# andabi/parallel-wavenet-vocoder

Hardware: AMD Instinct MI355X
Metric: audio samples/sec, 4-flow IAF generation (higher is better)
Workload: dtype f32 via 3-term split-fp16 MFMA (fp32 accumulate, fp32 storage)

## Files before the change

### parallel-wavenet-vocoder_amd/csrc/pwv_f16x3.h

```cpp
#pragma once

#include "pwv_layer_common.h"

namespace pwv {

typedef float f32x2 __attribute__((ext_vector_type(2)));

template <int OFF, int N>
__device__ __forceinline__ void split8(const float (&x)[N], f16x8& hi, f16x8& lo) {
#pragma unroll
    for (int q = 0; q < 8; q += 2) {
        const f32x2 v = {x[OFF + q], x[OFF + q + 1]};
        const f16x2 h = __builtin_convertvector(v, f16x2);
        f32x2 r;
        asm("v_fma_mix_f32 %0, %1, -1.0, %2 op_sel:[0,0,0] op_sel_hi:[1,0,0]" : "=v"(r[0]) : "v"(h), "v"(v[0]));
        asm("v_fma_mix_f32 %0, %1, -1.0, %2 op_sel:[1,0,0] op_sel_hi:[1,0,0]" : "=v"(r[1]) : "v"(h), "v"(v[1]));
        const f16x2 l = __builtin_convertvector(r, f16x2);
        hi[q] = h[0];
        hi[q + 1] = h[1];
        lo[q] = l[0];
        lo[q + 1] = l[1];
    }
}

// ... 48 lines not shown
        f16x8 nh[4] = {ah[0], ah[1], ah[2], ah[3]};
        f16x8 nl[4] = {al[0], al[1], al[2], al[3]};
        if (s + 1 < S1) {
#pragma unroll
            for (int i = 0; i < NIT; ++i) {
                nh[i] = frag16<NS, NITTOT>(A, 0, IT0 + i * ITSTEP, s + 1, lane);
                nl[i] = frag16<NS, NITTOT>(A, 1, IT0 + i * ITSTEP, s + 1, lane);
            }
        } else {
            tail(nh, nl);
        }
        __builtin_amdgcn_sched_barrier(0);
        const f16x8 b_h = bh(s);
        const f16x8 b_l = bl(s);
#pragma unroll
        for (int i = 0; i < NIT; ++i)
            acc[IT0 + i * ITSTEP] = __builtin_amdgcn_mfma_f32_32x32x16_f16(ah[i], b_h, acc[IT0 + i * ITSTEP], 0, 0, 0);
#pragma unroll
        for (int i = 0; i < NIT; ++i)
            acc[IT0 + i * ITSTEP] = __builtin_amdgcn_mfma_f32_32x32x16_f16(ah[i], b_l, acc[IT0 + i * ITSTEP], 0, 0, 0);
#pragma unroll
        for (int i = 0; i < NIT; ++i)
            acc[IT0 + i * ITSTEP] = __builtin_amdgcn_mfma_f32_32x32x16_f16(al[i], b_h, acc[IT0 + i * ITSTEP], 0, 0, 0);
        extra(s);
        __builtin_amdgcn_sched_barrier(0);
#pragma unroll
        for (int i = 0; i < 4; ++i) {
            ah[i] = nh[i];
            al[i] = nl[i];
        }
    }
}

template <int NS, int S, int NIT, int IT0, int ITSTEP, int NITTOT>
__device__ __forceinline__ void frags_at(const f16x8* A, int lane, f16x8 (&h)[4], f16x8 (&l)[4]) {
#pragma unroll
    for (int i = 0; i < NIT; ++i) {
        h[i] = frag16<NS, NITTOT>(A, 0, IT0 + i * ITSTEP, S, lane);
        l[i] = frag16<NS, NITTOT>(A, 1, IT0 + i * ITSTEP, S, lane);
    }
}

template <int NS, int NIT, int IT0, int ITSTEP, int NITTOT>
__device__ __forceinline__ void first_frags(const f16x8* A, int lane, f16x8 (&h)[4], f16x8 (&l)[4]) {
#pragma unroll
    for (int i = 0; i < NIT; ++i) {
        h[i] = frag16<NS, NITTOT>(A, 0, IT0 + i * ITSTEP, 0, lane);
        l[i] = frag16<NS, NITTOT>(A, 1, IT0 + i * ITSTEP, 0, lane);
    }
}

}
```

### parallel-wavenet-vocoder_amd/csrc/pwv_head_f16x3.inc

```
            f32x16 accs[4];
#pragma unroll
            for (int it = 0; it < 4; ++it)
#pragma unroll
                for (int q = 0; q < 4; ++q) {
                    const f32x4 v = *reinterpret_cast<const f32x4*>(hb + kHBS + h * 64 + it * 16 + q * 4);
#pragma unroll
                    for (int e = 0; e < 4; ++e) accs[it][q * 4 + e] = v[e];
                }
#pragma unroll
            for (int r = 0; r < 16; ++r) o[16 + r] = gate_act(acc[1][r], acc[3][r]);
            split8<16>(o, oh[2], ol[2]);
            split8<24>(o, oh[3], ol[3]);
            first_frags<4, 4, 0, 1, 4>(HS, lane, ah, al);
            gemm16<4, 4, 0, 1, 4>(HS, lane, accs, ah, al, [&](int s) -> f16x8 { return oh[s]; },
                                  [&](int s) -> f16x8 { return ol[s]; }, no_extra,
                                  [&](f16x8(&nh)[4], f16x8(&nl)[4]) { first_frags<8, 4, 0, 1, 4>(H1, lane, nh, nl); });
#pragma unroll
            for (int it = 0; it < 4; ++it)
#pragma unroll
                for (int q = 0; q < 4; ++q) {
                    const f32x4 v = *reinterpret_cast<const f32x4*>(hb + kHB1 + h * 64 + it * 16 + q * 4);
#pragma unroll
                    for (int e = 0; e < 4; ++e) acc1[it][q * 4 + e] = v[e];
                }
            f16x8 sh[8], sl[8];
            {
                float r[64];
#pragma unroll
                for (int i = 0; i < 64; ++i) r[i] = fmaxf(accs[i >> 4][i & 15], 0.f);
                split8<0>(r, sh[0], sl[0]);
                split8<8>(r, sh[1], sl[1]);
                split8<16>(r, sh[2], sl[2]);
                split8<24>(r, sh[3], sl[3]);
                split8<32>(r, sh[4], sl[4]);
                split8<40>(r, sh[5], sl[5]);
                split8<48>(r, sh[6], sl[6]);
                split8<56>(r, sh[7], sl[7]);
            }
            gemm16<8, 4, 0, 1, 4>(H1, lane, acc1, ah, al, [&](int s) -> f16x8 { return sh[s]; },
                                  [&](int s) -> f16x8 { return sl[s]; }, no_extra, [](f16x8(&)[4], f16x8(&)[4]) {});
```

### parallel-wavenet-vocoder_amd/csrc/pwv_head_pp2.inc

```
                    for (int q = 0; q < Q; ++q) {
                        float part = 0.f;
                        const float* w2 = hb + kHW2 + (hq + q) * 64;
#pragma unroll
                        for (int i4 = 0; i4 < 16; ++i4) {
                            const f32x4 wv = *reinterpret_cast<const f32x4*>(w2 + 4 * i4);
#pragma unroll
                            for (int e = 0; e < 4; ++e) {
                                const int i = 4 * i4 + e;
                                part = fmaf(fmaxf(acc1[i >> 4][i & 15], 0.f), wv[e], part);
                            }
                        }
                        part += __shfl_xor(part, 32);
                        part += hb[kHW2 + 2 * Q * 64 + q];
                        PWV_HEAD_STORE(q, part);
                    }
```

### parallel-wavenet-vocoder_amd/csrc/pwv_layer_f16x3_body.inc

```
    static_assert(!HEAD || (GATED && !SKIP && !COND && !FIRST), "HEAD: plain last layer only");
    static_assert(!FOLD || FIRST, "FOLD: layer 0 of a scalar-input net only");
    static_assert(!STREAM || (SKIP ? !COND && !FIRST && !HEAD : FOLD == FIRST && (COND ? !HEAD && !(FIRST && GATED) : GATED == HEAD)),
                  "STREAM: folded layer 0, plain residual layer, last layer + head; COND: the last layer gated, its head a launch of its own; "
                  "SKIP: a residual or gated layer on row histories (layer 0 behind a streaming front), the head a launch of its own");
    constexpr int WAVES = 8;
    constexpr int kLds = HEAD ? kA1Size + kASSize + kHA1Size : layer_floats(SKIP, COND);
    constexpr int kCF = kLds + 4;
    constexpr int kHS = kA1Size;
    constexpr int kH1 = kA1Size + kASSize;
    __shared__ __attribute__((aligned(16))) float lds[kLds + (HEAD ? 0 : 4) + (FIRST ? 128 : 0)];

    const int tid = threadIdx.x;
    const int lane = tid & 63;
    const int wave = __builtin_amdgcn_readfirstlane(tid >> 6);
    const int h = lane >> 5;
    const int net = blockIdx.x % p.G;
    const int wg = blockIdx.x / p.G;
    const int nwg = gridDim.x / p.G;
    int* unit_counter = reinterpret_cast<int*>(&lds[HEAD ? 0 : kLds]);
#ifdef PWV_TRACE
    if (p.trace && tid == 0) {
        p.trace[4096 + blockIdx.x * 4 + 0] = __builtin_amdgcn_s_memtime();
        p.trace[4096 + 1024 + blockIdx.x * 2 + 0] = __builtin_amdgcn_s_memrealtime();
    }
// ... 170 lines not shown
                    *reinterpret_cast<f32x4*>(hw + g * 256) = v;
                }
            }
        }
        auto split_xc = [&](int s) {
            if (s == 0) { split8<0>(xc, bh[4], bl[4]); asm volatile("" : "+v"(bh[4]), "+v"(bl[4])); }
            if (s == 1) { split8<8>(xc, bh[5], bl[5]); asm volatile("" : "+v"(bh[5]), "+v"(bl[5])); }
            if (s == 2) { split8<16>(xc, bh[6], bl[6]); asm volatile("" : "+v"(bh[6]), "+v"(bl[6])); }
            if (s == 3) { split8<24>(xc, bh[7], bl[7]); asm volatile("" : "+v"(bh[7]), "+v"(bl[7])); }
        };
        auto split_xb = [&](int s) {
            if (s == 0) { split8<0>(rxb, bh[0], bl[0]); asm volatile("" : "+v"(bh[0]), "+v"(bl[0])); }
            if (s == 1) { split8<8>(rxb, bh[1], bl[1]); asm volatile("" : "+v"(bh[1]), "+v"(bl[1])); }
            if (s == 2) { split8<16>(rxb, bh[2], bl[2]); asm volatile("" : "+v"(bh[2]), "+v"(bl[2])); }
            if (s == 3) { split8<24>(rxb, bh[3], bl[3]); asm volatile("" : "+v"(bh[3]), "+v"(bl[3])); }
        };
        if constexpr (!FOLD) {
#pragma unroll
            for (int s = 0; s < 4; ++s) {
                if constexpr (COND) split_xb(s);
                else split_xc(s);
            }
        }

        auto bxh = [&](int s) -> f16x8 { return bh[s ^ 4]; };
        auto bxl = [&](int s) -> f16x8 { return bl[s ^ 4]; };
        auto bch = [&](int s) -> f16x8 { return ch[COND ? s : 0]; };
        auto bcl = [&](int s) -> f16x8 { return cl[COND ? s : 0]; };

        PWV_STAMP(3);
        float o[32];
        f16x8 oh[4], ol[4];
        f16x8 ah[4], al[4];

        if constexpr (FOLD) {
            if constexpr (COND) {
                first_frags<5, 2, 0, 2, 4>(AC, lane, ah, al);
                gemm16<5, 2, 0, 2, 4>(AC, lane, acc, ah, al, bch, bcl, no_extra,
                                      [&](f16x8(&nh)[4], f16x8(&nl)[4]) { first_frags<5, 2, 1, 2, 4>(AC, lane, nh, nl); });
                gemm16<5, 2, 1, 2, 4>(AC, lane, acc, ah, al, bch, bcl, no_extra, [](f16x8(&)[4], f16x8(&)[4]) {});
            }
            const f16x8* F0 = reinterpret_cast<const f16x8*>(p.fold0[net]);
            f16x8 fh[4], fl[4];
#pragma unroll
            for (int it = 0; it < 4; ++it) {
                fh[it] = F0[it * 64 + lane];
                fl[it] = F0[(4 + it) * 64 + lane];
            }
#pragma unroll
            for (int it = 0; it < 4; ++it) acc[it] = __builtin_amdgcn_mfma_f32_32x32x16_f16(fh[it], fb_h, acc[it], 0, 0, 0);
#pragma unroll
            for (int it = 0; it < 4; ++it) acc[it] = __builtin_amdgcn_mfma_f32_32x32x16_f16(fh[it], fb_l, acc[it], 0, 0, 0);
#pragma unroll
            for (int it = 0; it < 4; ++it) acc[it] = __builtin_amdgcn_mfma_f32_32x32x16_f16(fl[it], fb_h, acc[it], 0, 0, 0);
            if constexpr (!GATED) first_frags<4, 2, 0, 1, 2>(A2, lane, ah, al);
#pragma unroll
            for (int r = 0; r < 16; ++r) o[r] = gate_act(acc[0][r], acc[2][r]);
            split8<0>(o, oh[0], ol[0]);
            split8<8>(o, oh[1], ol[1]);
        } else {
        if constexpr (COND) {
            first_frags<5, 2, 0, 2, 4>(AC, lane, ah, al);
            gemm16<5, 2, 0, 2, 4>(AC, lane, acc, ah, al, bch, bcl, split_xc,
                                  [&](f16x8(&nh)[4], f16x8(&nl)[4]) { first_frags<8, 2, 0, 2, 4>(A1, lane, nh, nl); });
        } else {
            first_frags<8, 2, 0, 2, 4>(A1, lane, ah, al);
        }
        gemm16<8, 2, 0, 2, 4>(
            A1, lane, acc, ah, al, bxh, bxl,
            [&](int s) {
                if constexpr (!COND) split_xb(s);
            },
            [&](f16x8(&nh)[4], f16x8(&nl)[4]) {
                if constexpr (COND) first_frags<5, 2, 1, 2, 4>(AC, lane, nh, nl);
                else first_frags<8, 2, 1, 2, 4>(A1, lane, nh, nl);
            });
        PWV_STAMP(4);
        if constexpr (COND) {
            gemm16<5, 2, 1, 2, 4>(AC, lane, acc, ah, al, bch, bcl, no_extra,
                                  [&](f16x8(&nh)[4], f16x8(&nl)[4]) { first_frags<8, 2, 1, 2, 4>(A1, lane, nh, nl); });
        }
        gemm16<8, 2, 1, 2, 4>(
            A1, lane, acc, ah, al, bxh, bxl,
            [&](int s) {
                o[2 * s] = gate_act(acc[0][2 * s], acc[2][2 * s]);
                o[2 * s + 1] = gate_act(acc[0][2 * s + 1], acc[2][2 * s + 1]);
                asm volatile("" : "+v"(o[2 * s]), "+v"(o[2 * s + 1]));
                if (s == 3) {
                    split8<0>(o, oh[0], ol[0]);
                    asm volatile("" : "+v"(oh[0]), "+v"(ol[0]));
                }
                if (s == 7) {
                    split8<8>(o, oh[1], ol[1]);
                    asm volatile("" : "+v"(oh[1]), "+v"(ol[1]));
                }
            },
            [&](f16x8(&nh)[4], f16x8(&nl)[4]) {
                if constexpr (!GATED) first_frags<4, 2, 0, 1, 2>(A2, lane, nh, nl);
                else if constexpr (SKIP) first_frags<4, 2, 0, 1, 4>(AS, lane, nh, nl);
            });
        }

        PWV_STAMP(5);
        const int ooff = units_off(row, h, 64, u_begin);
        if constexpr (GATED && HEAD) {
            const float* hb = p.packed_head[net];
            const f16x8* HS = reinterpret_cast<const f16x8*>(&lds[kHS]);
            const f16x8* H1 = reinterpret_cast<const f16x8*>(&lds[kH1]);
            f32x16 acc1[4];
#include "pwv_head_f16x3.inc"
            load_x(next, rxb, rxc);
            const int Q = p.head_q;
            const int hq = h * Q;
#define PWV_HEAD_STORE(q, part) if (valid && h == 0) p.head_out[net][(size_t)row * Q + (q)] = (part)
#include "pwv_head_pp2.inc"
#undef PWV_HEAD_STORE
        } else if constexpr (GATED) {
            if constexpr (!SKIP) load_x(next, rxb, rxc);
            __builtin_amdgcn_sched_barrier(0);
#pragma unroll
            for (int r = 0; r < 16; ++r) o[16 + r] = gate_act(acc[1][r], acc[3][r]);
            if constexpr (SKIP) {
                split8<16>(o, oh[2], ol[2]);
                split8<24>(o, oh[3], ol[3]);
            }
            if (valid) {
#pragma unroll
                for (int g = 0; g < 8; ++g) {
                    f32x4 v = {o[4 * g], o[4 * g + 1], o[4 * g + 2], o[4 * g + 3]};
                    store_wt(out_rs, ooff + g * 1024, v);
                }
            }
        } else {
            f32x16 acc2[2];
#pragma unroll
            for (int it = 0; it < 2; ++it)
#pragma unroll
                for (int q = 0; q < 4; ++q) {
                    const f32x4 bd = *reinterpret_cast<const f32x4*>(&lds[kBD + h * 32 + it * 16 + q * 4]);
#pragma unroll
                    for (int e = 0; e < 4; ++e) acc2[it][q * 4 + e] = xc[it * 16 + q * 4 + e] + bd[e];
                }
            asm volatile("" : "+v"(acc2[0]), "+v"(acc2[1]));
            if constexpr (!SKIP) load_x(next, rxb, rxc);
            __builtin_amdgcn_sched_barrier(0);
// ... 81 lines not shown
```

### parallel-wavenet-vocoder_amd/csrc/pwv_layer_f32_body.inc

```
    static_assert(!FOLD || FIRST, "FOLD: layer 0 of a scalar-input net only");
    static_assert(!STREAM || (SKIP ? !COND && !FIRST && !HEAD : FOLD == FIRST && (COND ? !HEAD && !(FIRST && GATED) : GATED == HEAD)),
                  "STREAM: folded layer 0, plain residual layer, last layer + head; COND: the last layer gated, its head a launch of its own; "
                  "SKIP: a residual or gated layer on row histories (layer 0 behind a streaming front), the head a launch of its own");
    static_assert(!HEAD || (GATED && !SKIP && !COND && !FIRST), "HEAD: plain last layer only");
    static_assert(!FIRST || !SKIP, "FIRST: no skip accumulation");
    constexpr int WAVES = 8;
    constexpr int kLds = HEAD ? kA1Size + kASSize + kHA1Size : layer_floats(SKIP, COND);
    constexpr int kCF = kLds + 4;
    constexpr int kHS = kA1Size;
    constexpr int kH1 = kA1Size + kASSize;
    __shared__ __attribute__((aligned(16))) float lds[kLds + (HEAD ? 0 : 4) + (FIRST ? 128 : 0)];

    const int tid = threadIdx.x;
    const int lane = tid & 63;
    const int wave = __builtin_amdgcn_readfirstlane(tid >> 6);
    const int h = lane >> 5;
    const int net = blockIdx.x % p.G;
    const int wg = blockIdx.x / p.G;
    const int nwg = gridDim.x / p.G;
    int* unit_counter = reinterpret_cast<int*>(&lds[HEAD ? 0 : kLds]);

    if constexpr (HEAD) {
        fill_lds_dma<kA1Size / 4, WAVES>(lds, p.packed[net] + kA1, wave, lane);
        fill_lds_dma<kASSize / 4, WAVES>(lds + kHS, p.packed_head[net] + kHAS, wave, lane);
// ... 140 lines not shown
                n[0] = frag(lds, kA1, 1, 16, 0, lane);
                n[1] = frag(lds, kA1, 3, 16, 0, lane);
            });
        }
        gemm_groups<16, 2, 1, 2>(
            lds, kA1, lane, acc, a, bx,
            [&](int g) {
                o[g] = gate_act(acc[0][g], acc[2][g]);
                asm volatile("" : "+v"(o[g]));
            },
            [&](f32x4(&n)[4]) {
                if constexpr (!GATED) {
                    n[0] = frag(lds, kA2, 0, 8, 0, lane);
                    n[1] = frag(lds, kA2, 1, 8, 0, lane);
                } else if constexpr (SKIP) {
#pragma unroll
                    for (int i = 0; i < 4; ++i) n[i] = frag(lds, kAS, i, 8, 0, lane);
                } else if constexpr (HEAD) {
#pragma unroll
                    for (int i = 0; i < 4; ++i) n[i] = frag(lds, kHS, i, 8, 0, lane);
                }
            });
        }

        const int ooff = units_off(cur.row, h, 64, u_begin);
        if constexpr (GATED && HEAD) {
            const float* hb = p.packed_head[net];
            f32x16 acc1[4];
#define PWV_HEAD_FENCE() do {} while (0)
#include "pwv_head_f32.inc"
#undef PWV_HEAD_FENCE
            const int Q = p.head_q;
            const int hq = h * Q;
#define PWV_HEAD_STORE(q, part) if (cur.valid && h == 0) p.head_out[net][(size_t)cur.row * Q + (q)] = (part)
#include "pwv_head_pp2.inc"
#undef PWV_HEAD_STORE
        } else if constexpr (GATED) {
            if constexpr (SKIP) load_skip_row<SKIP, COND>(p, net, lane, cur, skip_load);
#pragma unroll
            for (int r = 0; r < 16; ++r) o[16 + r] = gate_act(acc[1][r], acc[3][r]);
            if (cur.valid) {
#pragma unroll
                for (int g = 0; g < 8; ++g) {
                    f32x4 v = {o[4 * g], o[4 * g + 1], o[4 * g + 2], o[4 * g + 3]};
                    store_wt(out_rs, ooff + g * 1024, v);
                }
            }
        } else {
            f32x16 acc2[2];
#pragma unroll
            for (int it = 0; it < 2; ++it) {
#pragma unroll
                for (int q = 0; q < 4; ++q) {
                    const f32x4 bd = *reinterpret_cast<const f32x4*>(&lds[kBD + h * 32 + it * 16 + q * 4]);
                    if constexpr (FIRST) {
                        const int g = it * 4 + q;
                        const f32x4 w0 = *reinterpret_cast<const f32x4*>(&lds[kCF + 8 * g + 4 * h]);
                        const f32x4 w1 = *reinterpret_cast<const f32x4*>(&lds[kCF + 64 + 8 * g + 4 * h]);
#pragma unroll
                        for (int e = 0; e < 4; ++e) acc2[it][q * 4 + e] = fmaf(first_x0, w1[e], first_x1 * w0[e]) + bd[e];
                    } else {
#pragma unroll
                        for (int e = 0; e < 4; ++e) acc2[it][q * 4 + e] = cur.xc[it * 16 + q * 4 + e] + bd[e];
                    }
                }
            }
// ... 56 lines not shown
```

### parallel-wavenet-vocoder_amd/csrc/pwv_persist_tail.inc

```
    bool tail_done = false;
    {
        if (p.tail_q > 0) {
            tail_done = true;
            PT_EV(8, L, -1);
            __syncthreads();
            const int wg_dead = __builtin_amdgcn_readfirstlane(*(__attribute__((address_space(3))) volatile int*)&ctl[1]);
            __syncthreads();
            bool tail_ok = !wg_dead;
            if (tail_ok) {
                constexpr int kHS = kA1Size, kH1 = kA1Size + kASSize;
                fill_lds_dma<kA1Size / 4, 8>(lds, p.tail_layer[net] + kA1, wave, lane);
                fill_lds_dma<kASSize / 4, 8>(lds + kHS, p.tail_head[net] + kHAS, wave, lane);
                fill_lds_dma<kHA1Size / 4, 8>(lds + kH1, p.tail_head[net] + kHA1, wave, lane);
                const int td = p.tail_dil;
                if (w > 0 && wave < ((td + 31) >> 5)) {
                    const int w0 = w - p.tail_reach_wgs > 0 ? w - p.tail_reach_wgs : 0;
                    const int cnt = w - w0;
                    const long long t0 = __builtin_amdgcn_s_memrealtime();
                    for (int k = 0;; ++k) {
                        int v = 1 << 20;
                        if (lane < cnt) v = __hip_atomic_load(prog_n + (size_t)(w0 + lane) * kProgStride, __ATOMIC_RELAXED, __HIP_MEMORY_SCOPE_AGENT);
                        if (__ballot(v < L) == 0) break;
                        if ((k & 63) == 63 && (__builtin_amdgcn_readfirstlane(__hip_atomic_load(p.abort, __ATOMIC_RELAXED, __HIP_MEMORY_SCOPE_AGENT)) ||
                                               __builtin_amdgcn_s_memrealtime() - t0 > kWaitTicks)) {
                            __hip_atomic_store(p.status, 6, __ATOMIC_RELAXED, __HIP_MEMORY_SCOPE_SYSTEM);
                            __hip_atomic_store(p.abort, 1, __ATOMIC_RELAXED, __HIP_MEMORY_SCOPE_AGENT);
                            tail_ok = false;
                            break;
                        }
                        __builtin_amdgcn_s_sleep(4);
                    }
                }
                asm volatile("s_waitcnt vmcnt(0)" ::: "memory");
                __syncthreads();
                PT_EV(9, L, -1);
                const f16x8* A1 = reinterpret_cast<const f16x8*>(lds);
                const f16x8* HS = reinterpret_cast<const f16x8*>(lds + kHS);
                const f16x8* H1 = reinterpret_cast<const f16x8*>(lds + kH1);
                (void)A1; (void)HS; (void)H1;
                const float* hb = p.tail_head[net];
                const int Q = p.tail_q;
                const int so = in_soff(L);
                const __amdgpu_buffer_rsrc_t out_rs = [&]() {
                    const unsigned long long a = (unsigned long long)p.tail_out[net];
                    const unsigned lo = __builtin_amdgcn_readfirstlane((unsigned)a), hi2 = __builtin_amdgcn_readfirstlane((unsigned)(a >> 32));
                    return __builtin_amdgcn_make_buffer_rsrc((void*)(((unsigned long long)hi2 << 32) | lo), 0,
                                                             __builtin_amdgcn_readfirstlane((unsigned)rows * (unsigned)Q * 4u), 0x00020000);
                }();
                auto load_tail = [&](int unit, float (&xb)[32], float (&xc)[32]) {
                    int row, rc, nn, t;
                    bool valid;
                    rows_of(unit, row, valid, rc, nn, t);
                    const bool has_prev = t >= td;
                    const int oc = toff(rc), ob = toff(has_prev ? rc - td : rc);
#pragma unroll
                    for (int g = 0; g < 8; ++g) {
                        const f32x4 v = __builtin_bit_cast(f32x4, __builtin_amdgcn_raw_buffer_load_b128(ring_rs, oc + g * 1024, so, 16));
#pragma unroll
                        for (int e = 0; e < 4; ++e) xc[4 * g + e] = v[e];
                    }
#pragma unroll
                    for (int g = 0; g < 8; ++g) {
                        const f32x4 v = __builtin_bit_cast(f32x4, __builtin_amdgcn_raw_buffer_load_b128(ring_rs, ob + g * 1024, so, 16));
#pragma unroll
                        for (int e = 0; e < 4; ++e) xb[4 * g + e] = has_prev ? v[e] : 0.f;
                    }
                    hist_lookback(L, td, nn, t, unit, rc, xb);
                };
                auto no_extra = [](int) {};
                int unit = u_begin + wave;
                float txb[32], txc[32];
                load_tail(unit, txb, txc);
                while (tail_ok && unit < u_end) {
                    asm volatile("" ::: "memory");
                    const int next = unit + 8;
                    int row, rc, nn, t;
                    bool valid;
                    rows_of(unit, row, valid, rc, nn, t);
                    hist_store(L, td, nn, t, unit, rc, valid, txc);
                    f32x16 acc[4];
                    {
                        int prow = 0;
                        if (p.cond_hop > 0) prow = p_base(nn) + fast_div(t + p.cond_offset, p.hop_magic, p.hop_shift);
                        const float* pr = proj_n + (size_t)prow * p.proj_row_stride + L * 128 + h * 64;
#pragma unroll
                        for (int it = 0; it < 4; ++it)
#pragma unroll
                            for (int q = 0; q < 4; ++q) {
                                const f32x4 v = *reinterpret_cast<const f32x4*>(pr + it * 16 + q * 4);
#pragma unroll
                                for (int e = 0; e < 4; ++e) acc[it][q * 4 + e] = v[e];
                            }
                    }
                    f32x16 acc1[4];
                    if constexpr (F32) {
                        auto bx = [&](int ks) -> float { return ks < 32 ? txb[ks] : txc[ks - 32]; };
                        float o[32];
                        f32x4 a[4];
                        a[0] = frag(lds, 0, 0, 16, 0, lane);
                        a[1] = frag(lds, 0, 2, 16, 0, lane);
                        gemm_groups<16, 2, 0, 2>(lds, 0, lane, acc, a, bx, no_extra, [&](f32x4(&nf)[4]) {
                            nf[0] = frag(lds, 0, 1, 16, 0, lane);
                            nf[1] = frag(lds, 0, 3, 16, 0, lane);
                        });
                        gemm_groups<16, 2, 1, 2>(
                            lds, 0, lane, acc, a, bx,
                            [&](int g) {
                                o[g] = gate_act(acc[0][g], acc[2][g]);
                                asm volatile("" : "+v"(o[g]));
                            },
                            [&](f32x4(&nf)[4]) {
#pragma unroll
                                for (int i = 0; i < 4; ++i) nf[i] = frag(lds, kHS, i, 8, 0, lane);
                            });
#define PWV_HEAD_FENCE() asm volatile("" ::: "memory")
#include "pwv_head_f32.inc"
#undef PWV_HEAD_FENCE
                    } else {
                        f16x8 bh[8], bl[8];
                        float xc[32];
#pragma unroll
                        for (int i = 0; i < 32; ++i) xc[i] = txc[i];
                        split8<0>(xc, bh[4], bl[4]);
                        split8<8>(xc, bh[5], bl[5]);
                        split8<16>(xc, bh[6], bl[6]);
                        split8<24>(xc, bh[7], bl[7]);
                        auto bxh = [&](int s) -> f16x8 { return bh[s ^ 4]; };
                        auto bxl = [&](int s) -> f16x8 { return bl[s ^ 4]; };
                        float o[32];
                        f16x8 oh[4], ol[4];
                        f16x8 ah[4], al[4];
                        first_frags<8, 2, 0, 2, 4>(A1, lane, ah, al);
                        gemm16<8, 2, 0, 2, 4>(
                            A1, lane, acc, ah, al, bxh, bxl,
                            [&](int s) {
                                if (s == 0) { split8<0>(txb, bh[0], bl[0]); asm volatile("" : "+v"(bh[0]), "+v"(bl[0])); }
                                if (s == 1) { split8<8>(txb, bh[1], bl[1]); asm volatile("" : "+v"(bh[1]), "+v"(bl[1])); }
                                if (s == 2) { split8<16>(txb, bh[2], bl[2]); asm volatile("" : "+v"(bh[2]), "+v"(bl[2])); }
                                if (s == 3) { split8<24>(txb, bh[3], bl[3]); asm volatile("" : "+v"(bh[3]), "+v"(bl[3])); }
                            },
                            [&](f16x8(&nh)[4], f16x8(&nl)[4]) { first_frags<8, 2, 1, 2, 4>(A1, lane, nh, nl); });
                        gemm16<8, 2, 1, 2, 4>(
                            A1, lane, acc, ah, al, bxh, bxl,
                            [&](int s) {
                                o[2 * s] = gate_act(acc[0][2 * s], acc[2][2 * s]);
                                o[2 * s + 1] = gate_act(acc[0][2 * s + 1], acc[2][2 * s + 1]);
                                asm volatile("" : "+v"(o[2 * s]), "+v"(o[2 * s + 1]));
                                if (s == 3) { split8<0>(o, oh[0], ol[0]); asm volatile("" : "+v"(oh[0]), "+v"(ol[0])); }
                                if (s == 7) { split8<8>(o, oh[1], ol[1]); asm volatile("" : "+v"(oh[1]), "+v"(ol[1])); }
                            },
                            [](f16x8(&)[4], f16x8(&)[4]) {});
#include "pwv_head_f16x3.inc"
                    }
                    load_tail(next, txb, txc);
                    float outv[kMaxQ] = {0.f, 0.f, 0.f, 0.f};
                    int out_idx = row * Q, hq = h * Q;
                    asm volatile("" : "+v"(out_idx), "+v"(hq));
#define PWV_HEAD_STORE(q, part) do { if ((q) < kMaxQ) outv[q] = (part); \
         \
        if (valid && h == 0) __builtin_amdgcn_raw_buffer_store_b32(__builtin_bit_cast(unsigned, (part)), out_rs, (out_idx + (q)) * 4, 0, kAuxWriteThrough); } while (0)
#include "pwv_head_pp2.inc"
#undef PWV_HEAD_STORE
                    if (p.affine_x && p.G == 1 && Q == 2) {
                        if (valid && h == 0) p.affine_out[row] = fmaf(p.affine_x[row], outv[0], outv[1]);
                    }
                    __builtin_amdgcn_sched_barrier(0);
                    PT_EV(10, L, unit);
                    unit = next;
                }
            }
            asm volatile("s_waitcnt vmcnt(0)" ::: "memory");
            __syncthreads();
            if (p.affine_x && p.pair && p.G == 2) {
                if (tid == 0) {
                    const int old = __hip_atomic_fetch_add(p.pair + w, 1, __ATOMIC_RELAXED, __HIP_MEMORY_SCOPE_AGENT);
                    *(__attribute__((address_space(3))) volatile int*)&ctl[0] = old;
                }
                __syncthreads();
                const int old = __builtin_amdgcn_readfirstlane(*(__attribute__((address_space(3))) volatile int*)&ctl[0]);
                if (old == 1) {
                    const int r_end = u_end * 32 < rows ? u_end * 32 : rows;
                    for (int row = u_begin * 32 + tid; row < r_end; row += 512) {
                        const float sv = __hip_atomic_load(p.tail_out[0] + row, __ATOMIC_RELAXED, __HIP_MEMORY_SCOPE_AGENT);
                        const float bv = __hip_atomic_load(p.tail_out[1] + row, __ATOMIC_RELAXED, __HIP_MEMORY_SCOPE_AGENT);
                        p.affine_out[row] = fmaf(p.affine_x[row], sv, bv);
                    }
                    if (tid == 0) __hip_atomic_store(p.pair + w, 0, __ATOMIC_RELAXED, __HIP_MEMORY_SCOPE_AGENT);
                }
            }
            asm volatile("s_waitcnt vmcnt(0)" ::: "memory");
            __syncthreads();
            PT_EV(11, L, -1);
            if (wave == 0) {
                int done = 0;
                if (lane == 0) done = __hip_atomic_fetch_add(p.exited, 1, __ATOMIC_RELAXED, __HIP_MEMORY_SCOPE_AGENT);
                if (__builtin_amdgcn_readfirstlane(done) == p.active_wgs - 1) {
                    for (int k = lane; k < p.G * p.nwg; k += 64) __hip_atomic_store(p.prog + (size_t)k * kProgStride, 0, __ATOMIC_RELAXED, __HIP_MEMORY_SCOPE_AGENT);
                    if (SHORT) for (int k = lane; k < p.G * p.units; k += 64) __hip_atomic_store(p.uprog + (size_t)k * kUnitStride, 0, __ATOMIC_RELAXED, __HIP_MEMORY_SCOPE_AGENT);
                    if (lane == 0) {
                        __hip_atomic_store(p.abort, 0, __ATOMIC_RELAXED, __HIP_MEMORY_SCOPE_AGENT);
                        __hip_atomic_store(p.exited, 0, __ATOMIC_RELAXED, __HIP_MEMORY_SCOPE_AGENT);
                    }
// ... 5 lines not shown
```

### parallel-wavenet-vocoder_amd/csrc/pwv_stack_persist.hip

```cpp
#include "pwv_f16x3.h"
#include "pwv_persist_plan.h"

#include <cstddef>
#include <cstdlib>
#include <cstring>

namespace pwv {

constexpr int kStoreAuxLocal = 0;

constexpr int kSlotFull = kA1Size + kA2Size;
constexpr int kSlot = kSlotFull - 256;
constexpr int kBiasF = 2 * kSlot;
constexpr int kCtlF = kBiasF + 128;
constexpr int kCtlInts = 40;
constexpr int kLdsFloats = 40960;
constexpr int kCfF = kCtlF + kCtlInts;
constexpr int kLeftB = (kCfF + 128) * 4;
constexpr int kDoneB = kLeftB + kLeftN;
constexpr int kMaxUnitsWgLds = kLdsFloats * 4 - kDoneB;
static_assert(kMaxUnitsWg == kMaxUnitsWgLds && kPlanMaxQ == kMaxQ, "pwv_persist_plan.h restates the kernel's limits");
static_assert(kUnitModeMaxPerWg <= 7, "the short-input instantiation keeps wave 7 as its loader");
static_assert(kLeftN <= 32, "unit mode: the right neighbours are polled by lanes 32..63 alone");
constexpr int kFlagB = (kCtlF + 2) * 4;
// ... 11 lines not shown
    int* abort;
    int* exited;
    int active_wgs;
    int* status;
    long long packed_stride;
    int proj_row_stride;
    int G, N, T, n_layers, units, per_wg, nwg, last_wg, reach_wgs, xcd_map, rot;
    int all_wt;
    int cond_hop, cond_offset, cond_frames;
    unsigned T_magic, T_shift, hop_magic, hop_shift;
    int dil[kMaxPLayers];
    const float* x_first;
    const float* cfilt[PWV_MAX_NETS];
    const float* fold0[PWV_MAX_NETS];
    float x_limit;
    int* range_flag;
    long long* trace;
    long long* trace_ev;
    const float* tail_layer[PWV_MAX_NETS];
    const float* tail_head[PWV_MAX_NETS];
    float* tail_out[PWV_MAX_NETS];
    int tail_q, tail_dil, tail_reach_wgs;
    const float* affine_x;
    float* affine_out;
    int* pair;
    const int* unit_map;
    const float* hist_rd;
    float* hist_wr;
    const int* slot_tab;
    long long hist_block_stride;
    long long hist_scalar_off;
    long long hist_off[PWV_MAX_NETS][kMaxPLayers + 1];
    const int* cu_rows;
};

#ifdef PWV_PTRACE
#define PT_DECL long long pt_acc[18] = {0, 0, 0, 0, 0, 0, 0, 0, 0, 0, 0, 0, 0, 0, 0, 0, 0, 0}; long long pt_t = 0, pt_p = 0; (void)pt_t; (void)pt_p;
#define PT_BEGIN() pt_t = __builtin_amdgcn_s_memtime()
#define PT_END(k) pt_acc[k] += __builtin_amdgcn_s_memtime() - pt_t
#define PT_ADD(k, v) pt_acc[k] += (v)
#define PT_LAP(k) do { __builtin_amdgcn_sched_barrier(0); const long long pt_n = __builtin_amdgcn_s_memtime(); pt_acc[k] += pt_n - pt_t; pt_t = pt_n; __builtin_amdgcn_sched_barrier(0); } while (0)
#define PT_MARK() do { __builtin_amdgcn_sched_barrier(0); pt_p = __builtin_amdgcn_s_memtime(); __builtin_amdgcn_sched_barrier(0); } while (0)
#define PT_PHASE(k) do { __builtin_amdgcn_sched_barrier(0); const long long pt_n = __builtin_amdgcn_s_memtime(); pt_acc[k] += pt_n - pt_p; pt_p = pt_n; __builtin_amdgcn_sched_barrier(0); } while (0)
#define PT_EV(code, jj, uu) do { if (p.trace_ev && pt_nev < 64) { if (lane == 0) { long long* e_ = p.trace_ev + (((size_t)blockIdx.x * 8 + wave) * 64 + pt_nev) * 4; \
    e_[0] = __builtin_amdgcn_s_memrealtime(); e_[1] = (code); e_[2] = (jj); e_[3] = (long long)(uu); } ++pt_nev; } } while (0)
#else
#define PT_DECL
#define PT_BEGIN() do {} while (0)
#define PT_END(k) do {} while (0)
#define PT_ADD(k, v) do {} while (0)
#define PT_LAP(k) do {} while (0)
#define PT_MARK() do {} while (0)
#define PT_PHASE(k) do {} while (0)
#define PT_EV(code, jj, uu) do {} while (0)
#endif

constexpr unsigned kRawMask = 0xFu, kWarMask = 0x30u;

template <typename FR, typename BH, typename BL, typename EF>
__device__ __forceinline__ void gemm16_dense(FR&& fr, f32x16 (&acc)[2], f16x8 (&ah)[4], f16x8 (&al)[4], BH&& bh, BL&& bl, EF&& extra) {
#pragma unroll
    for (int s = 0; s < 4; ++s) {
        f16x8 nh[2] = {ah[0], ah[1]};
        f16x8 nl[2] = {al[0], al[1]};
        if (s + 1 < 4) {
#pragma unroll
            for (int i = 0; i < 2; ++i) {
                nh[i] = fr(0, i, s + 1);
                nl[i] = fr(1, i, s + 1);
            }
        }
        __builtin_amdgcn_sched_barrier(0);
        const f16x8 b_h = bh(s);
        const f16x8 b_l = bl(s);
#pragma unroll
        for (int i = 0; i < 2; ++i) acc[i] = __builtin_amdgcn_mfma_f32_32x32x16_f16(ah[i], b_h, acc[i], 0, 0, 0);
#pragma unroll
        for (int i = 0; i < 2; ++i) acc[i] = __builtin_amdgcn_mfma_f32_32x32x16_f16(ah[i], b_l, acc[i], 0, 0, 0);
#pragma unroll
        for (int i = 0; i < 2; ++i) acc[i] = __builtin_amdgcn_mfma_f32_32x32x16_f16(al[i], b_h, acc[i], 0, 0, 0);
        extra(s);
        __builtin_amdgcn_sched_barrier(0);
#pragma unroll
        for (int i = 0; i < 2; ++i) {
            ah[i] = nh[i];
            al[i] = nl[i];
        }
// ... 285 lines not shown
            PWV_CHECK_ARG(a->affine_out && ((a->G == 2 && a->tail_q == 1) || (a->G == 1 && a->tail_q == 2)),
                          "pwv_wavenet_stack_persist_f32: the fused affine needs affine_out and (G = 2, tail_q = 1) or (G = 1, tail_q = 2)");
            p.affine_x = a->affine_x;
            p.affine_out = a->affine_out;
            p.pair = pair_words;
        }
    } else {
        PWV_CHECK_ARG(!a->affine_x, "pwv_wavenet_stack_persist_f32: affine_x without a tail");
    }
    (void)pair_words;
    if (streaming) {
        p.hist_rd = sa.hist_rd;
        p.hist_wr = sa.hist_wr;
        p.slot_tab = sa.slot_tab;
        p.hist_block_stride = (long long)sa.block_stride;
        p.hist_scalar_off = (long long)sa.scalar_off;
        PWV_CHECK_ARG(!a->x_first || sa.scalar_off + (size_t)a->dilations[0] + 1 <= sa.block_stride,
                      "pwv_wavenet_stack_persist_f32: hist->scalar_off + dilation + 1 scalars leave the history block");
        const int n_hist = a->n_layers + (a->tail_q > 0 ? 1 : 0);
        for (int g = 0; g < a->G; ++g)
            for (int j = a->x_first ? 1 : 0; j < n_hist; ++j) {
                const size_t off = a->hist_row_off[g][j];
                const size_t hist_rows = ((size_t)(j < a->n_layers ? a->dilations[j] : a->tail_dilation) + 31) / 32 * 32;
                PWV_CHECK_ARG(off % 4 == 0 && off + hist_rows * 64 <= sa.block_stride,
                              "pwv_wavenet_stack_persist_f32: hist_row_off[%d][%d] + round32(dilation) rows leave the history block", g, j);
                p.hist_off[g][j] = (long long)off;
            }
    }
    p.trace = nullptr;
#ifdef PWV_PTRACE
    { const char* e = getenv("PWV_PTRACE_PTR"); if (e) p.trace = (long long*)strtoull(e, nullptr, 0); }
    p.trace_ev = nullptr;
    { const char* e = getenv("PWV_PTRACE_EV_PTR"); if (e) p.trace_ev = (long long*)strtoull(e, nullptr, 0); }
#endif
    hipStream_t s = (hipStream_t)stream;
    const size_t n16 = r.lay.total / 16;
    if (!a->workspace_clean)
        hipLaunchKernelGGL(persist_zero_kernel, dim3((unsigned)((n16 + 255) / 256)), dim3(256), 0, s, (int4*)a->workspace, n16);
    const dim3 grid(a->G * pl.nwg), block(512);
    const persist_kernel_t kernel = (ragged ? kRagged : streaming ? kStreaming : varlen ? kPacked : kUniform)[a->precision == PWV_PREC_F32][pl.unit_mode == 2];
    hipLaunchKernelGGL(kernel, grid, block, 0, s, p);
    hipError_t e = hipGetLastError();
    if (e != hipSuccess) return set_error(PWV_EHIP, "persistent stack kernel launch failed: %s", hipGetErrorString(e));
    return PWV_OK;
}

int pwv_varlen_unit_map(const int* cu_rows, const int* cu_frames, int n_utt, int units, int* out, pwv_stream_t stream) {
    PWV_CHECK_ARG(cu_rows && out, "pwv_varlen_unit_map: NULL argument");
    PWV_CHECK_ARG(n_utt >= 1 && units >= 1, "pwv_varlen_unit_map: n_utt = %d, units = %d", n_utt, units);
    PWV_CHECK_ARG(((uintptr_t)out & 15) == 0, "pwv_varlen_unit_map: out must be 16-byte aligned");
    hipLaunchKernelGGL(varlen_unit_map_kernel, dim3((unsigned)((units + 255) / 256)), dim3(256), 0, (hipStream_t)stream, cu_rows, cu_frames, n_utt, units, out);
    hipError_t e = hipGetLastError();
    if (e != hipSuccess) return set_error(PWV_EHIP, "pwv_varlen_unit_map launch failed: %s", hipGetErrorString(e));
    return PWV_OK;
}

}
```

Before: 60.54 million.

## Interleave head gating, splits, bias loads and pp2 dot into MFMA schedule groups

Rewrites the f16x3 head path so the gate activation, hi/lo fp16 splitting, ReLU splits, bias tile loads and part of the pp2 output dot product run inside the MFMA issue stream. A new gemm16g helper uses sched_group_barrier. The skip-bias load and first head fragment fetch are moved into the preceding GEMM's extra and tail hooks. The first 48 pp2 terms for q==0 are computed during the last GEMM, and the rest of pp2 skips them. The aim is to hide VALU and LDS latency behind MFMAs, at the cost of register pressure and fragile hand scheduling. Tail-trace timing macros are also added, but they compile away unless PWV_PTRACE is defined.

```diff
diff --git a/parallel-wavenet-vocoder_amd/csrc/pwv_f16x3.h b/parallel-wavenet-vocoder_amd/csrc/pwv_f16x3.h
--- a/parallel-wavenet-vocoder_amd/csrc/pwv_f16x3.h
+++ b/parallel-wavenet-vocoder_amd/csrc/pwv_f16x3.h
@@ -104,6 +104,72 @@
     }
 }
 
+template <int N>
+__device__ __forceinline__ void split2(const float (&x)[N], int off, int q, f16x8& hi, f16x8& lo) {
+    const f32x2 v = {x[off], x[off + 1]};
+    const f16x2 h = __builtin_convertvector(v, f16x2);
+    f32x2 r;
+    asm("v_fma_mix_f32 %0, %1, -1.0, %2 op_sel:[0,0,0] op_sel_hi:[1,0,0]" : "=v"(r[0]) : "v"(h), "v"(v[0]));
+    asm("v_fma_mix_f32 %0, %1, -1.0, %2 op_sel:[1,0,0] op_sel_hi:[1,0,0]" : "=v"(r[1]) : "v"(h), "v"(v[1]));
+    const f16x2 l = __builtin_convertvector(r, f16x2);
+    hi[q] = h[0];
+    hi[q + 1] = h[1];
+    lo[q] = l[0];
+    lo[q + 1] = l[1];
+}
+
+template <int S0, int KS, int IT0, int NIT, bool TILE_MAJOR, int HALF, int NACC, typename BH, typename BL, typename SF>
+__device__ __forceinline__ void gemm16g(f32x16 (&acc)[NACC], f16x8 (&ah)[4], f16x8 (&al)[4], BH&& bh, BL&& bl, SF&& step) {
+    static_assert(NIT * KS <= 4 && IT0 + NIT <= NACC, "a group holds four fragment pairs at most");
+    constexpr int NM = 3 * NIT * KS;
+    static_assert(NM % 2 == 0, "MFMAs go in twos");
+    f16x8 nh[4] = {ah[0], ah[1], ah[2], ah[3]};
+    f16x8 nl[4] = {al[0], al[1], al[2], al[3]};
+    __builtin_amdgcn_sched_barrier(0);
+#pragma unroll
+    for (int m = 0; m < NM; ++m) {
+        const int i = TILE_MAJOR ? m / (3 * KS) : m % NIT;
+        const int k = TILE_MAJOR ? (m / 3) % KS : m / (3 * NIT);
+        const int c = TILE_MAJOR ? m % 3 : (m / NIT) % 3;
+        acc[IT0 + i] = __builtin_amdgcn_mfma_f32_32x32x16_f16(c == 2 ? al[i * KS + k] : ah[i * KS + k], c == 1 ? bl(S0 + k) : bh(S0 + k), acc[IT0 + i], 0, 0, 0);
+        if (m % 2 == 1) {
+            step(m / 2, nh, nl);
+            __builtin_amdgcn_sched_group_barrier(0x008, 1, 0);
+            __builtin_amdgcn_sched_group_barrier(0x522, HALF, 0);
+            __builtin_amdgcn_sched_group_barrier(0x008, 1, 0);
+            __builtin_amdgcn_sched_group_barrier(0x522, 12, 0);
+            __builtin_amdgcn_sched_barrier(0);
+        }
+    }
+#pragma unroll
+    for (int i = 0; i < 4; ++i) {
+        ah[i] = nh[i];
+        al[i] = nl[i];
+    }
+}
+
+template <int NS, int NITTOT, int S0, int KS, int IT0, int NIT>
+__device__ __forceinline__ void frags_slot(const f16x8* A, int lane, int slot, f16x8 (&h)[4], f16x8 (&l)[4]) {
+    static_assert(NIT * KS <= 4, "a group holds four fragment pairs at most");
+#pragma unroll
+    for (int i = 0; i < NIT; ++i)
+#pragma unroll
+        for (int k = 0; k < KS; ++k)
+            if (slot == i * KS + k) {
+                h[slot] = frag16<NS, NITTOT>(A, 0, IT0 + i, S0 + k, lane);
+                l[slot] = frag16<NS, NITTOT>(A, 1, IT0 + i, S0 + k, lane);
+            }
+}
+
+__device__ __forceinline__ void bias_tile(const float* src, f32x16& a) {
+#pragma unroll
+    for (int q = 0; q < 4; ++q) {
+        const f32x4 v = *reinterpret_cast<const f32x4*>(src + q * 4);
+#pragma unroll
+        for (int e = 0; e < 4; ++e) a[q * 4 + e] = v[e];
+    }
+}
+
 template <int NS, int S, int NIT, int IT0, int ITSTEP, int NITTOT>
 __device__ __forceinline__ void frags_at(const f16x8* A, int lane, f16x8 (&h)[4], f16x8 (&l)[4]) {
 #pragma unroll
diff --git a/parallel-wavenet-vocoder_amd/csrc/pwv_head_f16x3.inc b/parallel-wavenet-vocoder_amd/csrc/pwv_head_f16x3.inc
--- a/parallel-wavenet-vocoder_amd/csrc/pwv_head_f16x3.inc
+++ b/parallel-wavenet-vocoder_amd/csrc/pwv_head_f16x3.inc
@@ -1,41 +1,98 @@
-            f32x16 accs[4];
+            auto obh = [&](int s) -> f16x8 { return oh[s]; };
+            auto obl = [&](int s) -> f16x8 { return ol[s]; };
+            auto gate1 = [&](int r) {
+                o[16 + r] = gate_act(acc[1][r], acc[3][r]);
+                asm volatile("" : "+v"(o[16 + r]));
+            };
+            auto osplit = [&](int p) {
+                split2(o, 16 + 2 * p, (2 * p) & 7, oh[2 + p / 4], ol[2 + p / 4]);
+                if (p % 4 == 3) asm volatile("" : "+v"(oh[2 + p / 4]), "+v"(ol[2 + p / 4]));
+            };
+            f16x8 sh[8], sl[8];
+            auto rsplit = [&](int s, int j) {
+                const float r[2] = {fmaxf(accs[s >> 1][8 * (s & 1) + 2 * j], 0.f), fmaxf(accs[s >> 1][8 * (s & 1) + 2 * j + 1], 0.f)};
+                split2(r, 0, 2 * j, sh[s], sl[s]);
+                if (j == 3) asm volatile("" : "+v"(sh[s]), "+v"(sl[s]));
+            };
+            gemm16g<0, 1, 0, 4, false, 6>(accs, ah, al, obh, obl, [&](int m, f16x8(&nh)[4], f16x8(&nl)[4]) {
+                frags_slot<4, 4, 1, 1, 0, 4>(HS, lane, m, nh, nl);
+                gate1(m);
+            });
+            gemm16g<1, 1, 0, 4, false, 6>(accs, ah, al, obh, obl, [&](int m, f16x8(&nh)[4], f16x8(&nl)[4]) {
+                frags_slot<4, 4, 2, 1, 0, 4>(HS, lane, m, nh, nl);
+                if (m < 2) gate1(6 + m);
+                else if (m < 4) { osplit(2 * m - 4); osplit(2 * m - 3); }
+                else gate1(4 + m);
+            });
+            gemm16g<2, 1, 0, 4, false, 6>(accs, ah, al, obh, obl, [&](int m, f16x8(&nh)[4], f16x8(&nl)[4]) {
+                frags_slot<4, 4, 3, 1, 0, 4>(HS, lane, m, nh, nl);
+                gate1(10 + m);
+                if (m == 1 || m == 2) osplit(3 + m);
+                if (m == 4 || m == 5) osplit(2 + m);
+            });
+            gemm16g<3, 1, 0, 4, true, 5>(accs, ah, al, obh, obl, [&](int m, f16x8(&nh)[4], f16x8(&nl)[4]) {
+                frags_slot<8, 4, 0, 1, 0, 4>(H1, lane, m, nh, nl);
+                if (m < 2) {
+                    bias_tile(hb + kHB1 + h * 64 + 32 * m, acc1[2 * m]);
+                    bias_tile(hb + kHB1 + h * 64 + 32 * m + 16, acc1[2 * m + 1]);
+                } else {
+                    rsplit(0, m - 2);
+                }
+            });
+            auto sbh = [&](int s) -> f16x8 { return sh[s]; };
+            auto sbl = [&](int s) -> f16x8 { return sl[s]; };
+            int hq0 = h * Q;
+            asm volatile("" : "+v"(hq0));
+            const float* w20 = hb + kHW2 + hq0 * 64;
+            f32x4 w2a[4], w2b[4], w2c[4];
+            auto pp2_w = [&](int it, f32x4(&w)[4]) {
 #pragma unroll
-            for (int it = 0; it < 4; ++it)
+                for (int q4 = 0; q4 < 4; ++q4) w[q4] = *reinterpret_cast<const f32x4*>(w20 + it * 16 + 4 * q4);
+            };
+            auto pp2_terms = [&](int it, int e0, int e1, const f32x4(&w)[4]) {
 #pragma unroll
-                for (int q = 0; q < 4; ++q) {
-                    const f32x4 v = *reinterpret_cast<const f32x4*>(hb + kHBS + h * 64 + it * 16 + q * 4);
-#pragma unroll
-                    for (int e = 0; e < 4; ++e) accs[it][q * 4 + e] = v[e];
-                }
-#pragma unroll
-            for (int r = 0; r < 16; ++r) o[16 + r] = gate_act(acc[1][r], acc[3][r]);
-            split8<16>(o, oh[2], ol[2]);
-            split8<24>(o, oh[3], ol[3]);
-            first_frags<4, 4, 0, 1, 4>(HS, lane, ah, al);
-            gemm16<4, 4, 0, 1, 4>(HS, lane, accs, ah, al, [&](int s) -> f16x8 { return oh[s]; },
-                                  [&](int s) -> f16x8 { return ol[s]; }, no_extra,
-                                  [&](f16x8(&nh)[4], f16x8(&nl)[4]) { first_frags<8, 4, 0, 1, 4>(H1, lane, nh, nl); });
-#pragma unroll
-            for (int it = 0; it < 4; ++it)
-#pragma unroll
-                for (int q = 0; q < 4; ++q) {
-                    const f32x4 v = *reinterpret_cast<const f32x4*>(hb + kHB1 + h * 64 + it * 16 + q * 4);
-#pragma unroll
-                    for (int e = 0; e < 4; ++e) acc1[it][q * 4 + e] = v[e];
-                }
-            f16x8 sh[8], sl[8];
-            {
-                float r[64];
-#pragma unroll
-                for (int i = 0; i < 64; ++i) r[i] = fmaxf(accs[i >> 4][i & 15], 0.f);
-                split8<0>(r, sh[0], sl[0]);
-                split8<8>(r, sh[1], sl[1]);
-                split8<16>(r, sh[2], sl[2]);
-                split8<24>(r, sh[3], sl[3]);
-                split8<32>(r, sh[4], sl[4]);
-                split8<40>(r, sh[5], sl[5]);
-                split8<48>(r, sh[6], sl[6]);
-                split8<56>(r, sh[7], sl[7]);
-            }
-            gemm16<8, 4, 0, 1, 4>(H1, lane, acc1, ah, al, [&](int s) -> f16x8 { return sh[s]; },
-                                  [&](int s) -> f16x8 { return sl[s]; }, no_extra, [](f16x8(&)[4], f16x8(&)[4]) {});
+                for (int e = 0; e < 16; ++e)
+                    if (e >= e0 && e < e1) part0 = fmaf(fmaxf(acc1[it][e], 0.f), w[e >> 2][e & 3], part0);
+                asm volatile("" : "+v"(part0));
+            };
+            gemm16g<0, 1, 0, 4, false, 5>(acc1, ah, al, sbh, sbl, [&](int m, f16x8(&nh)[4], f16x8(&nl)[4]) {
+                frags_slot<8, 4, 1, 1, 0, 4>(H1, lane, m, nh, nl);
+                if (m < 4) rsplit(1, m);
+            });
+            gemm16g<1, 1, 0, 4, false, 5>(acc1, ah, al, sbh, sbl, [&](int m, f16x8(&nh)[4], f16x8(&nl)[4]) {
+                frags_slot<8, 4, 2, 1, 0, 4>(H1, lane, m, nh, nl);
+                if (m < 4) rsplit(2, m);
+            });
+            gemm16g<2, 1, 0, 4, false, 5>(acc1, ah, al, sbh, sbl, [&](int m, f16x8(&nh)[4], f16x8(&nl)[4]) {
+                frags_slot<8, 4, 3, 1, 0, 4>(H1, lane, m, nh, nl);
+                if (m < 4) rsplit(3, m);
+            });
+            gemm16g<3, 1, 0, 4, false, 5>(acc1, ah, al, sbh, sbl, [&](int m, f16x8(&nh)[4], f16x8(&nl)[4]) {
+                frags_slot<8, 4, 4, 1, 0, 4>(H1, lane, m, nh, nl);
+                if (m < 4) rsplit(4, m);
+            });
+            gemm16g<4, 1, 0, 4, false, 9>(acc1, ah, al, sbh, sbl, [&](int m, f16x8(&nh)[4], f16x8(&nl)[4]) {
+                frags_slot<8, 4, 5, 1, 0, 4>(H1, lane, m, nh, nl);
+                if (m < 4) rsplit(5, m);
+                if (m >= 2) rsplit(6, m - 2);
+            });
+            gemm16g<5, 1, 0, 4, false, 6>(acc1, ah, al, sbh, sbl, [&](int m, f16x8(&nh)[4], f16x8(&nl)[4]) {
+                frags_slot<8, 4, 6, 2, 0, 1>(H1, lane, m, nh, nl);
+                if (m < 4) rsplit(7, m);
+                if (m == 4) pp2_w(0, w2a);
+            });
+            part0 = 0.f;
+            gemm16g<6, 2, 0, 1, true, 9>(acc1, ah, al, sbh, sbl, [&](int m, f16x8(&nh)[4], f16x8(&nl)[4]) {
+                frags_slot<8, 4, 6, 2, 1, 1>(H1, lane, m, nh, nl);
+                if (m == 1) pp2_w(1, w2b);
+                if (m == 2) pp2_w(2, w2c);
+            });
+            gemm16g<6, 2, 1, 1, true, 9>(acc1, ah, al, sbh, sbl, [&](int m, f16x8(&nh)[4], f16x8(&nl)[4]) {
+                frags_slot<8, 4, 6, 2, 2, 1>(H1, lane, m, nh, nl);
+                pp2_terms(0, m == 0 ? 0 : 5 * m + 1, 5 * m + 6, w2a);
+            });
+            gemm16g<6, 2, 2, 1, true, 9>(acc1, ah, al, sbh, sbl, [&](int m, f16x8(&nh)[4], f16x8(&nl)[4]) {
+                frags_slot<8, 4, 6, 2, 3, 1>(H1, lane, m, nh, nl);
+                pp2_terms(1, m == 0 ? 0 : 5 * m + 1, 5 * m + 6, w2b);
+            });
+            gemm16g<6, 2, 3, 1, true, 9>(acc1, ah, al, sbh, sbl, [&](int m, f16x8(&)[4], f16x8(&)[4]) { pp2_terms(2, m == 0 ? 0 : 5 * m + 1, 5 * m + 6, w2c); });
diff --git a/parallel-wavenet-vocoder_amd/csrc/pwv_head_pp2.inc b/parallel-wavenet-vocoder_amd/csrc/pwv_head_pp2.inc
--- a/parallel-wavenet-vocoder_amd/csrc/pwv_head_pp2.inc
+++ b/parallel-wavenet-vocoder_amd/csrc/pwv_head_pp2.inc
@@ -1,8 +1,19 @@
                     for (int q = 0; q < Q; ++q) {
-                        float part = 0.f;
+                        float part = q == 0 ? part0 : 0.f;
                         const float* w2 = hb + kHW2 + (hq + q) * 64;
+                        if (pp2_done > 0 && q > 0) {
 #pragma unroll
-                        for (int i4 = 0; i4 < 16; ++i4) {
+                            for (int i4 = 0; i4 < pp2_done / 4; ++i4) {
+                                const f32x4 wv = *reinterpret_cast<const f32x4*>(w2 + 4 * i4);
+#pragma unroll
+                                for (int e = 0; e < 4; ++e) {
+                                    const int i = 4 * i4 + e;
+                                    part = fmaf(fmaxf(acc1[i >> 4][i & 15], 0.f), wv[e], part);
+                                }
+                            }
+                        }
+#pragma unroll
+                        for (int i4 = pp2_done / 4; i4 < 16; ++i4) {
                             const f32x4 wv = *reinterpret_cast<const f32x4*>(w2 + 4 * i4);
 #pragma unroll
                             for (int e = 0; e < 4; ++e) {
diff --git a/parallel-wavenet-vocoder_amd/csrc/pwv_layer_f16x3_body.inc b/parallel-wavenet-vocoder_amd/csrc/pwv_layer_f16x3_body.inc
--- a/parallel-wavenet-vocoder_amd/csrc/pwv_layer_f16x3_body.inc
+++ b/parallel-wavenet-vocoder_amd/csrc/pwv_layer_f16x3_body.inc
@@ -226,6 +226,9 @@
         float o[32];
         f16x8 oh[4], ol[4];
         f16x8 ah[4], al[4];
+        static_assert(!(HEAD && FOLD), "HEAD: the skip bias is requested under the general GEMM1");
+        f32x16 accs[HEAD ? 4 : 1];
+        (void)accs;
 
         if constexpr (FOLD) {
             if constexpr (COND) {
@@ -288,10 +291,13 @@
                     split8<8>(o, oh[1], ol[1]);
                     asm volatile("" : "+v"(oh[1]), "+v"(ol[1]));
                 }
+                if constexpr (GATED && HEAD)
+                    if (s >= 4) bias_tile(p.packed_head[net] + kHBS + h * 64 + (s - 4) * 16, accs[s - 4]);
             },
             [&](f16x8(&nh)[4], f16x8(&nl)[4]) {
                 if constexpr (!GATED) first_frags<4, 2, 0, 1, 2>(A2, lane, nh, nl);
                 else if constexpr (SKIP) first_frags<4, 2, 0, 1, 4>(AS, lane, nh, nl);
+                else if constexpr (HEAD) first_frags<4, 4, 0, 1, 4>(reinterpret_cast<const f16x8*>(&lds[kHS]), lane, nh, nl);
             });
         }
 
@@ -302,9 +308,11 @@
             const f16x8* HS = reinterpret_cast<const f16x8*>(&lds[kHS]);
             const f16x8* H1 = reinterpret_cast<const f16x8*>(&lds[kH1]);
             f32x16 acc1[4];
+            float part0 = 0.f;
+            constexpr int pp2_done = 48;
+            const int Q = p.head_q;
 #include "pwv_head_f16x3.inc"
             load_x(next, rxb, rxc);
-            const int Q = p.head_q;
             const int hq = h * Q;
 #define PWV_HEAD_STORE(q, part) if (valid && h == 0) p.head_out[net][(size_t)row * Q + (q)] = (part)
 #include "pwv_head_pp2.inc"
diff --git a/parallel-wavenet-vocoder_amd/csrc/pwv_layer_f32_body.inc b/parallel-wavenet-vocoder_amd/csrc/pwv_layer_f32_body.inc
--- a/parallel-wavenet-vocoder_amd/csrc/pwv_layer_f32_body.inc
+++ b/parallel-wavenet-vocoder_amd/csrc/pwv_layer_f32_body.inc
@@ -196,6 +196,8 @@
 #undef PWV_HEAD_FENCE
             const int Q = p.head_q;
             const int hq = h * Q;
+            constexpr int pp2_done = 0;
+            constexpr float part0 = 0.f;
 #define PWV_HEAD_STORE(q, part) if (cur.valid && h == 0) p.head_out[net][(size_t)cur.row * Q + (q)] = (part)
 #include "pwv_head_pp2.inc"
 #undef PWV_HEAD_STORE
diff --git a/parallel-wavenet-vocoder_amd/csrc/pwv_persist_tail.inc b/parallel-wavenet-vocoder_amd/csrc/pwv_persist_tail.inc
--- a/parallel-wavenet-vocoder_amd/csrc/pwv_persist_tail.inc
+++ b/parallel-wavenet-vocoder_amd/csrc/pwv_persist_tail.inc
@@ -34,6 +34,9 @@
                 asm volatile("s_waitcnt vmcnt(0)" ::: "memory");
                 __syncthreads();
                 PT_EV(9, L, -1);
+                TT_DECL
+                TT_SET(4, __builtin_amdgcn_s_memtime());
+                TT_SET(5, __builtin_amdgcn_s_memrealtime());
                 const f16x8* A1 = reinterpret_cast<const f16x8*>(lds);
                 const f16x8* HS = reinterpret_cast<const f16x8*>(lds + kHS);
                 const f16x8* H1 = reinterpret_cast<const f16x8*>(lds + kH1);
@@ -73,6 +76,7 @@
                 load_tail(unit, txb, txc);
                 while (tail_ok && unit < u_end) {
                     asm volatile("" ::: "memory");
+                    TT_BEGIN();
                     const int next = unit + 8;
                     int row, rc, nn, t;
                     bool valid;
@@ -93,6 +97,8 @@
                             }
                     }
                     f32x16 acc1[4];
+                    float part0 = 0.f;
+                    constexpr int pp2_done = F32 ? 0 : 48;
                     if constexpr (F32) {
                         auto bx = [&](int ks) -> float { return ks < 32 ? txb[ks] : txc[ks - 32]; };
                         float o[32];
@@ -140,6 +146,7 @@
                                 if (s == 3) { split8<24>(txb, bh[3], bl[3]); asm volatile("" : "+v"(bh[3]), "+v"(bl[3])); }
                             },
                             [&](f16x8(&nh)[4], f16x8(&nl)[4]) { first_frags<8, 2, 1, 2, 4>(A1, lane, nh, nl); });
+                        f32x16 accs[4];
                         gemm16<8, 2, 1, 2, 4>(
                             A1, lane, acc, ah, al, bxh, bxl,
                             [&](int s) {
@@ -148,9 +155,12 @@
                                 asm volatile("" : "+v"(o[2 * s]), "+v"(o[2 * s + 1]));
                                 if (s == 3) { split8<0>(o, oh[0], ol[0]); asm volatile("" : "+v"(oh[0]), "+v"(ol[0])); }
                                 if (s == 7) { split8<8>(o, oh[1], ol[1]); asm volatile("" : "+v"(oh[1]), "+v"(ol[1])); }
+                                if (s >= 4) bias_tile(hb + kHBS + h * 64 + (s - 4) * 16, accs[s - 4]);
                             },
-                            [](f16x8(&)[4], f16x8(&)[4]) {});
+                            [&](f16x8(&nh)[4], f16x8(&nl)[4]) { first_frags<4, 4, 0, 1, 4>(HS, lane, nh, nl); });
+                        TT_LAP(0);
 #include "pwv_head_f16x3.inc"
+                        TT_LAP(1);
                     }
                     load_tail(next, txb, txc);
                     float outv[kMaxQ] = {0.f, 0.f, 0.f, 0.f};
@@ -166,8 +176,13 @@
                     }
                     __builtin_amdgcn_sched_barrier(0);
                     PT_EV(10, L, unit);
+                    TT_LAP(2);
+                    TT_SET(3, tt_acc[3] + 1);
                     unit = next;
                 }
+                TT_SET(6, __builtin_amdgcn_s_memtime());
+                TT_SET(7, __builtin_amdgcn_s_memrealtime());
+                TT_DUMP();
             }
             asm volatile("s_waitcnt vmcnt(0)" ::: "memory");
             __syncthreads();
diff --git a/parallel-wavenet-vocoder_amd/csrc/pwv_stack_persist.hip b/parallel-wavenet-vocoder_amd/csrc/pwv_stack_persist.hip
--- a/parallel-wavenet-vocoder_amd/csrc/pwv_stack_persist.hip
+++ b/parallel-wavenet-vocoder_amd/csrc/pwv_stack_persist.hip
@@ -67,6 +67,9 @@
     long long hist_scalar_off;
     long long hist_off[PWV_MAX_NETS][kMaxPLayers + 1];
     const int* cu_rows;
+#ifdef PWV_PTRACE
+    long long* trace_tail;
+#endif
 };
 
 #ifdef PWV_PTRACE
@@ -77,6 +80,11 @@
 #define PT_LAP(k) do { __builtin_amdgcn_sched_barrier(0); const long long pt_n = __builtin_amdgcn_s_memtime(); pt_acc[k] += pt_n - pt_t; pt_t = pt_n; __builtin_amdgcn_sched_barrier(0); } while (0)
 #define PT_MARK() do { __builtin_amdgcn_sched_barrier(0); pt_p = __builtin_amdgcn_s_memtime(); __builtin_amdgcn_sched_barrier(0); } while (0)
 #define PT_PHASE(k) do { __builtin_amdgcn_sched_barrier(0); const long long pt_n = __builtin_amdgcn_s_memtime(); pt_acc[k] += pt_n - pt_p; pt_p = pt_n; __builtin_amdgcn_sched_barrier(0); } while (0)
+#define TT_DECL long long tt_acc[8] = {0, 0, 0, 0, 0, 0, 0, 0}; long long tt_t = 0; (void)tt_t;
+#define TT_BEGIN() do { __builtin_amdgcn_sched_barrier(0); tt_t = __builtin_amdgcn_s_memtime(); __builtin_amdgcn_sched_barrier(0); } while (0)
+#define TT_LAP(k) do { __builtin_amdgcn_sched_barrier(0); const long long tt_n = __builtin_amdgcn_s_memtime(); tt_acc[k] += tt_n - tt_t; tt_t = tt_n; __builtin_amdgcn_sched_barrier(0); } while (0)
+#define TT_SET(k, v) tt_acc[k] = (v)
+#define TT_DUMP() do { if (p.trace_tail && lane == 0) { long long* t_ = p.trace_tail + ((size_t)blockIdx.x * 8 + wave) * 8; for (int k_ = 0; k_ < 8; ++k_) t_[k_] = tt_acc[k_]; } } while (0)
 #define PT_EV(code, jj, uu) do { if (p.trace_ev && pt_nev < 64) { if (lane == 0) { long long* e_ = p.trace_ev + (((size_t)blockIdx.x * 8 + wave) * 64 + pt_nev) * 4; \
     e_[0] = __builtin_amdgcn_s_memrealtime(); e_[1] = (code); e_[2] = (jj); e_[3] = (long long)(uu); } ++pt_nev; } } while (0)
 #else
@@ -88,6 +96,11 @@
 #define PT_MARK() do {} while (0)
 #define PT_PHASE(k) do {} while (0)
 #define PT_EV(code, jj, uu) do {} while (0)
+#define TT_DECL
+#define TT_BEGIN() do {} while (0)
+#define TT_LAP(k) do {} while (0)
+#define TT_SET(k, v) do {} while (0)
+#define TT_DUMP() do {} while (0)
 #endif
 
 constexpr unsigned kRawMask = 0xFu, kWarMask = 0x30u;
@@ -439,6 +452,8 @@
     { const char* e = getenv("PWV_PTRACE_PTR"); if (e) p.trace = (long long*)strtoull(e, nullptr, 0); }
     p.trace_ev = nullptr;
     { const char* e = getenv("PWV_PTRACE_EV_PTR"); if (e) p.trace_ev = (long long*)strtoull(e, nullptr, 0); }
+    p.trace_tail = nullptr;
+    { const char* e = getenv("PWV_PTRACE_TAIL_PTR"); if (e) p.trace_tail = (long long*)strtoull(e, nullptr, 0); }
 #endif
     hipStream_t s = (hipStream_t)stream;
     const size_t n16 = r.lay.total / 16;
```

Measured after the change: 61.01 million (median of 6 runs). About the same (+0.8%).
